# fritzsedlazeck/Sniffles

Measured on NVIDIA H100. Metric: aligned long-read Gbp/s through lead->cluster->consensus, higher is better.
Workload: dtype int32

## Files before the change

sniffles_b200/csrc/api.cu:

```cuda
#include <algorithm>
#include <climits>
#include <cstdio>
#include <cstdlib>
#include <cstring>
#include <string>
#include <vector>
#include <dlfcn.h>
#include <omp.h>

#include "common.cuh"
#include "prims.cuh"
#include "extract.cuh"
#include "cluster.cuh"
#include "consensus.cuh"
#include "poa.cuh"
#include "combine.cuh"
#include "population.cuh"
#include "ingest.cuh"
#include "bgzf_write.cuh"
#include "genotype.cuh"
#include "rnames.cuh"
#include "reference.cuh"

template <bool Pinned> struct Buf {
// ... 53 lines not shown

struct Caps { unsigned long long lead = 0, cand = 0, cand_lead = 0, rn = 0, alt = 0, scr16 = 0, item = 0, tile = 0, req = 0, req16 = 0; };

struct snfb_ctx {
    int device = 0; cudaStream_t st = nullptr, st_copy = nullptr, st_side = nullptr; cudaEvent_t ev_b = nullptr, ev_mid = nullptr, ev_fork = nullptr, ev_join = nullptr; std::string err;
    cudaEvent_t ev_aligned[consensus::MAX_SLICES] = {}, ev_slice[consensus::MAX_SLICES] = {}; int n_slices = consensus::DEFAULT_SLICES;
    snfb_config cfg{}; bool have_cfg = false;
    bool loaded = false, on_device = false, seq_on_demand = false; const uint8_t* h_seq = nullptr; uint32_t evt_min = 0;
    uint64_t n_rec = 0, n_cigar = 0, n_var = 0, n_seq = 0; uint32_t n_task = 0, n_contig = 0, n_tr = 0, n_mask = 0;
    const snfb_rec* d_rec = nullptr; const uint16_t* d_cigar = nullptr; const uint8_t* d_var = nullptr; const uint8_t* d_seq = nullptr;
    DevBuf b_rec, b_cigar, b_var, b_seq, b_task, b_contig, b_tr, b_trp, b_mask, b_mask_off, b_mask_task;
    HostBuf h_c16, h_rec16;
    DevBuf b_comp, b_raw, b_ing, b_ing_work; HostBuf h_ing; uint64_t ing_sizes[8] = {0, 0, 0, 0, 0, 0, 0, 0}; bool from_bam = false;
    DevBuf b_zin, b_zslot, b_zout, b_zwork;
    DevBuf b_gt;
    DevBuf b_rn, b_rn_text; HostBuf h_rn_meta, h_rn_text;
    DevBuf b_pop, b_popq; population::P pop{}; bool have_pop = false;
    DevBuf b_ref, b_ref_work; std::vector<refseq::Contig> ref_ctg; bool have_ref = false;
    HostBuf h_ref_runs, h_ref_coff, h_ref_out; uint64_t ref_n_runs = 0;
    std::vector<snfb_task> tasks;
    std::vector<snfb_region> regions, next_regions; DevBuf b_region; uint32_t n_region = 0; bool cov_view = false;
    Caps cap; bool force_no_cuts = false;
    DevBuf b_ctr, arena_r, arena_l, arena_c;
    int32_t* rec_pos; int32_t* rec_end; uint8_t* rec_flags; double* rec_nm; uint32_t* rec_nlead; uint32_t* rec_lead_off; uint32_t* sa_list; extract::RecScan* scanrec; extract::RecClip* clip; int32_t* rec_big;
    uint32_t* task_first; uint32_t* task_last; uint32_t* task_reads; unsigned long long* task_cov; int32_t* task_span; double* task_nm; double* nm_part; unsigned* nm_cnt; extract::Seg* sa_seg; uint32_t* scan_tmp_r;
    int32_t* v_pos; int32_t* v_end; uint8_t* v_flags; uint64_t* v_k0; uint64_t* v_k1; uint32_t* v_v0; uint32_t* v_v1; uint32_t* v_hist; uint32_t* v_scan; unsigned long long* v_n;
    snfb_lead* leads; extract::Event* ev_buf; snfb_lead* sorted_leads; uint32_t* radix_hist;
    cluster::B B{};
    consensus::C Cc{}; consensus::SeqReq* seq_req; uint32_t* arena_off; uint8_t* seq_arena; uint32_t* q_scan_tmp;
    HostBuf h_seq_req, h_seq_arena; uint64_t seq_h2d_bytes = 0;
    bool stage_a_done = false, stage_b_done = false, stage_c_done = false;
    HostBuf h_ctr_buf; DevCounters* h_mid = nullptr; DevCounters* h_fin = nullptr; consensus::Work* h_work = nullptr;
    HostBuf h_leads, h_task_reads, h_task_nm, h_rec_nm, h_cand, h_cand_leads, h_rnames, h_rn_off, h_task_cov, h_task_cov_raw, h_alt, h_cov_bins;
    void* comm = nullptr; int rank = 0, nranks = 1; DevBuf b_gsend, b_grecv; HostBuf h_gather, h_gather_out; unsigned long long gather_cap = 0;
    cudaEvent_t ev[MAX_TIMINGS + 1]; const char* ev_name[MAX_TIMINGS + 1]; uint64_t ev_bytes[MAX_TIMINGS + 1]; int n_ev = 0; int n_ev_load = 0; uint64_t launches = 0; uint64_t reruns = 0;
};

static uint32_t evt_need(const snfb_ctx* ctx) {
    if (!ctx->have_cfg) return SNFB_CIGAR16_EVT_MIN;
    int t = ctx->cfg.minsvlen_screen < 1 ? 1 : ctx->cfg.minsvlen_screen;
    if ((ctx->cfg.qc_nm_measure || ctx->cfg.phase) && t > 11) t = 11;
    return (uint32_t)(t < (int)SNFB_CIGAR16_EVT_MIN ? t : (int)SNFB_CIGAR16_EVT_MIN);
}
static void ctx_fail(snfb_ctx* ctx, const char* what, const char* msg) { ctx->err = std::string(what) + ": " + msg; }
static int fail(snfb_ctx* ctx, const std::string& m) { ctx->err = m; return 1; }

static void mark(snfb_ctx* ctx, const char* name, uint64_t bytes = 0) {
    if (ctx->n_ev >= MAX_TIMINGS) return;
    cudaEventRecord(ctx->ev[ctx->n_ev], ctx->st);
    ctx->ev_name[ctx->n_ev] = name; ctx->ev_bytes[ctx->n_ev] = bytes; ++ctx->n_ev;
}
static int grid_for(unsigned long long n, int threads) { unsigned long long g = (n + threads - 1) / threads; if (g < 1) g = 1; if (g > (uint64_t)NUM_SMS * 32) g = (uint64_t)NUM_SMS * 32; return (int)g; }
static int bits_for(uint32_t n) { int b = 0; while ((1ull << b) < n) ++b; return b; }

__global__ void k_gather_leads(const snfb_lead* __restrict__ leads, const uint32_t* __restrict__ sval, snfb_lead* __restrict__ out, const unsigned long long* n_ptr, unsigned long long cap) {
    const unsigned long long n = *n_ptr < cap ? *n_ptr : cap;
    for (unsigned long long i = blockIdx.x * (unsigned long long)blockDim.x + threadIdx.x; i < n; i += (unsigned long long)gridDim.x * blockDim.x) out[i] = leads[sval[i]];
}
__global__ void k_view_keys(const snfb_rec* __restrict__ rec, const int32_t* __restrict__ rec_pos, unsigned long long n, uint64_t* __restrict__ key, uint32_t* __restrict__ val, unsigned long long* n_out) {
    for (unsigned long long i = blockIdx.x * (unsigned long long)blockDim.x + threadIdx.x; i < n; i += (unsigned long long)gridDim.x * blockDim.x) {
        key[i] = ((uint64_t)(uint32_t)__ldg(&rec[i].task) << 32) | (uint64_t)((uint32_t)rec_pos[i] ^ 0x80000000u); val[i] = (uint32_t)i;
    }
    if (blockIdx.x == 0 && threadIdx.x == 0) *n_out = n;
}
__global__ void k_view_gather(const uint32_t* __restrict__ ord, unsigned long long n, const int32_t* __restrict__ pos, const int32_t* __restrict__ end, const uint8_t* __restrict__ flags,
                              int32_t* __restrict__ v_pos, int32_t* __restrict__ v_end, uint8_t* __restrict__ v_flags) {
    for (unsigned long long i = blockIdx.x * (unsigned long long)blockDim.x + threadIdx.x; i < n; i += (unsigned long long)gridDim.x * blockDim.x) {
        const uint32_t j = ord[i]; v_pos[i] = pos[j]; v_end[i] = end[j]; v_flags[i] = flags[j];
    }
}
__global__ void k_cov_bins(const int32_t* __restrict__ rec_pos, const int32_t* __restrict__ rec_end, const uint8_t* __restrict__ rec_flags, uint32_t lo, uint32_t hi,
                           int binsize, long long contig_len, long long nbins, unsigned long long* __restrict__ acc) {
    for (unsigned long long i = lo + blockIdx.x * (unsigned long long)blockDim.x + threadIdx.x; i < hi; i += (unsigned long long)gridDim.x * blockDim.x) {
        if (!(rec_flags[i] & extract::RF_PASS)) continue;
        long long a = rec_pos[i], e = rec_end[i]; if (a < 0) a = 0; if (e > contig_len) e = contig_len;
        if (e <= a) continue;
        for (long long bb = a / binsize; bb <= (e - 1) / binsize && bb < nbins; ++bb) {
            const long long s0 = bb * binsize, s1 = s0 + binsize;
            const long long o0 = a > s0 ? a : s0, o1 = e < s1 ? e : s1;
            if (o1 > o0) atomicAdd(&acc[bb], (unsigned long long)(o1 - o0));
        }
    }
}


struct GatherHdr { unsigned long long n_cand, n_alt, n_rn, n_leads, need_bytes, overflow, pad0, pad1; };
__host__ __device__ inline void gather_offsets(const GatherHdr& h, unsigned long long off[6]) {
    auto al = [](unsigned long long x) { return (x + 15ull) & ~15ull; };
    off[0] = sizeof(GatherHdr); off[1] = al(off[0] + h.n_cand * sizeof(snfb_cand)); off[2] = al(off[1] + h.n_alt); off[3] = al(off[2] + 8 * h.n_rn);
    off[4] = al(off[3] + 4 * h.n_cand); off[5] = al(off[4] + h.n_leads * sizeof(snfb_lead));
}
// ... 479 lines not shown
    CUDA_TRY(cudaStreamSynchronize(st));
    ctx->loaded = true; ctx->from_bam = true; return 0;
}

int snfb_ingest_sizes(snfb_ctx* ctx, uint64_t out[8]) {
    if (!ctx || !out || !ctx->from_bam) return 1;
    for (int i = 0; i < 8; ++i) out[i] = ctx->ing_sizes[i];
    return 0;
}
int snfb_ingest_fetch(snfb_ctx* ctx, snfb_rec* rec, uint16_t* cigar16, uint8_t* var, uint8_t* seq) {
    if (!ctx || !ctx->from_bam || !ctx->loaded) return ctx ? fail(ctx, "snfb_ingest_fetch: no block built by snfb_load_bam") : 1;
    cudaSetDevice(ctx->device);
    if (rec && ctx->n_rec) CUDA_TRY(cudaMemcpy(rec, ctx->d_rec, sizeof(snfb_rec) * ctx->n_rec, cudaMemcpyDeviceToHost));
    if (cigar16 && ctx->n_cigar) CUDA_TRY(cudaMemcpy(cigar16, ctx->d_cigar, 2 * ctx->n_cigar, cudaMemcpyDeviceToHost));
    if (var && ctx->n_var) CUDA_TRY(cudaMemcpy(var, ctx->d_var, ctx->n_var, cudaMemcpyDeviceToHost));
    if (seq && ctx->n_seq) CUDA_TRY(cudaMemcpy(seq, ctx->d_seq, ctx->n_seq, cudaMemcpyDeviceToHost));
    return 0;
}

}

static void carve_r(snfb_ctx* ctx, Carver& c) {
    const size_t n = ctx->n_rec + 1, nt = ctx->n_task;
    ctx->rec_pos = c.take<int32_t>(n); ctx->rec_end = c.take<int32_t>(n); ctx->rec_flags = c.take<uint8_t>(n); ctx->rec_nm = c.take<double>(n); ctx->rec_nlead = c.take<uint32_t>(n); ctx->rec_lead_off = c.take<uint32_t>(n);
    ctx->sa_list = c.take<uint32_t>(n); ctx->scanrec = c.take<extract::RecScan>(n); ctx->clip = c.take<extract::RecClip>(n); ctx->rec_big = c.take<int32_t>(n);
    ctx->task_first = c.take<uint32_t>(nt); ctx->task_last = c.take<uint32_t>(nt); ctx->task_reads = c.take<uint32_t>(nt); ctx->task_cov = c.take<unsigned long long>(nt); ctx->task_span = c.take<int32_t>(nt); ctx->task_nm = c.take<double>(nt);
    const size_t cpt = (ctx->n_rec + extract::NM_CHUNK - 1) / extract::NM_CHUNK + 1;
    ctx->nm_part = c.take<double>(cpt * nt + 1); ctx->nm_cnt = c.take<unsigned>(cpt * nt + 1);
    ctx->sa_seg = c.take<extract::Seg>((size_t)extract::MAXSEG * extract::SA_THREADS * extract::SA_BLOCKS);
    ctx->scan_tmp_r = c.take<uint32_t>(prims::scan_tmp_elems(n) + 16);
    const size_t nv = ctx->cov_view ? n : 1;
    ctx->v_pos = c.take<int32_t>(nv); ctx->v_end = c.take<int32_t>(nv); ctx->v_flags = c.take<uint8_t>(nv);
    ctx->v_k0 = c.take<uint64_t>(nv); ctx->v_k1 = c.take<uint64_t>(nv); ctx->v_v0 = c.take<uint32_t>(nv); ctx->v_v1 = c.take<uint32_t>(nv);
    ctx->v_hist = c.take<uint32_t>(prims::radix_hist_elems(nv) + 16); ctx->v_scan = c.take<uint32_t>(prims::scan_tmp_elems(std::max<size_t>(nv, prims::radix_hist_elems(nv))) + 16);
    ctx->v_n = c.take<unsigned long long>(1);
}
static void carve_l(snfb_ctx* ctx, Carver& c) {
    const size_t n = (size_t)ctx->cap.lead + 8; cluster::B& b = ctx->B;
    ctx->leads = c.take<snfb_lead>(n); ctx->ev_buf = c.take<extract::Event>(n); ctx->sorted_leads = c.take<snfb_lead>(n);
    b.key0 = c.take<uint64_t>(n); b.val0 = c.take<uint32_t>(n); b.key1 = c.take<uint64_t>(n); b.val1 = c.take<uint32_t>(n); b.flag = c.take<uint32_t>(n); b.scan = c.take<uint32_t>(n);
    b.scan_tmp = c.take<uint32_t>(prims::scan_tmp_elems(std::max<unsigned long long>(n, prims::radix_hist_elems(n))) + 16);
    ctx->radix_hist = c.take<uint32_t>(prims::radix_hist_elems(n) + 16);
    b.bin_start = c.take<uint32_t>(n); b.bin_nl = c.take<uint32_t>(n); b.bin_nlong = c.take<uint32_t>(n); b.bin_kept = c.take<uint32_t>(n); b.bin_hap = c.take<uint32_t>(3 * n);
    b.kl_off = c.take<uint32_t>(n); b.kll_off = c.take<uint32_t>(n); b.kb_idx = c.take<uint32_t>(n); b.kl = c.take<uint32_t>(n); b.kll = c.take<uint32_t>(n); b.kleads = c.take<snfb_lead>(n); b.klleads = c.take<snfb_lead>(n);
    b.kb_bin = c.take<uint32_t>(n); b.kb_lead_off = c.take<uint32_t>(n); b.kb_lead_n = c.take<uint32_t>(n); b.kb_long_off = c.take<uint32_t>(n); b.kb_long_n = c.take<uint32_t>(n); b.kb_seed = c.take<int32_t>(n); b.kb_chain = c.take<uint32_t>(n); b.kb_repeat = c.take<uint8_t>(n);
    b.seg_start = c.take<uint32_t>(n); b.c_next = c.take<uint32_t>(n); b.c_last = c.take<uint32_t>(n); b.c_sd = c.take<double>(n); b.c_mean = c.take<double>(n); b.c_rep = c.take<uint8_t>(n);
    b.seg_sd_last = c.take<double>(n); b.seg_maxsd_first = c.take<double>(n); b.cl_first = c.take<uint32_t>(n); b.cl_last = c.take<uint32_t>(n); b.cl_rep = c.take<uint8_t>(n); b.big_list = c.take<uint32_t>(n); b.mid_list = c.take<uint32_t>(n);
// ... 5 lines not shown
static void carve_c(snfb_ctx* ctx, Carver& c) {
    const Caps& k = ctx->cap; cluster::B& b = ctx->B; consensus::C& cc = ctx->Cc;
    b.cand = c.take<snfb_cand>(k.cand + 1); b.cand_leads = c.take<snfb_lead>(k.cand_lead + 1); b.out_plo = c.take<uint32_t>(k.cand_lead + 1); b.out_pn = c.take<uint32_t>(k.cand_lead + 1);
    b.rnames = c.take<uint64_t>(k.rn + 1); b.rn_off_out = c.take<uint32_t>(k.cand + 2);
    cc.plan_best = c.take<uint32_t>(k.cand + 1); cc.plan_nother = c.take<uint32_t>(k.cand + 1); cc.plan_otot = c.take<uint32_t>(k.cand + 1); cc.alt_len = c.take<uint32_t>(k.cand + 1); cc.scr_len = c.take<uint32_t>(k.cand + 1);
    cc.alt_off = c.take<uint32_t>(k.cand + 1); cc.scr_off = c.take<uint32_t>(k.cand + 1); cc.work_big = c.take<uint32_t>(k.cand + 1); cc.work_small = c.take<uint32_t>(k.cand + 1); cc.work = c.take<consensus::Work>(1);
    cc.q_cnt = c.take<uint32_t>(consensus::NQ * (k.cand + 1)); cc.q_off = c.take<uint32_t>(consensus::NQ * (k.cand + 1)); ctx->q_scan_tmp = c.take<uint32_t>(consensus::NQ * prims::scan_tmp_elems(k.cand));
    cc.items_big = c.take<consensus::C::Item>(k.item + 1); cc.items_small = c.take<consensus::C::Item>(k.item + 1); cc.tiles = c.take<uint2>(k.tile + 1);
    cc.alt = c.take<uint8_t>(k.alt + 64); cc.scr = c.take<uint8_t>(k.scr16 * 16 + 64);
    ctx->seq_req = c.take<consensus::SeqReq>(k.req + 1); ctx->seq_arena = c.take<uint8_t>(k.req16 * 16 + 64);
}
static int ensure_arenas(snfb_ctx* ctx) {
    if (carve(ctx->arena_r, [&](Carver& c) { carve_r(ctx, c); })) return fail(ctx, "out of device memory (per-record arrays)");
    if (carve(ctx->arena_l, [&](Carver& c) { carve_l(ctx, c); })) return fail(ctx, "out of device memory (per-lead arrays)");
    if (carve(ctx->arena_c, [&](Carver& c) { carve_c(ctx, c); })) return fail(ctx, "out of device memory (candidate / consensus arrays)");
    return 0;
}

static void bind_inputs(snfb_ctx* ctx) {
    cluster::B& b = ctx->B;
    b.leads = ctx->leads; b.rec = ctx->d_rec; b.task = ctx->b_task.as<snfb_task>(); b.contig = ctx->b_contig.as<snfb_contig>();
    b.tr = ctx->n_tr ? ctx->b_tr.as<int32_t>() : nullptr; b.tr_pmax = ctx->b_trp.as<int32_t>();
    b.rec_pos = ctx->cov_view ? ctx->v_pos : ctx->rec_pos; b.rec_end = ctx->cov_view ? ctx->v_end : ctx->rec_end; b.rec_flags = ctx->cov_view ? ctx->v_flags : ctx->rec_flags; b.rec_nm = ctx->rec_nm; b.rec_nlead = ctx->rec_nlead; b.rec_lead_off = ctx->rec_lead_off;
    b.task_first = ctx->task_first; b.task_last = ctx->task_last; b.task_maxspan = ctx->task_span;
    b.mask = ctx->n_mask ? ctx->b_mask.as<int32_t>() : nullptr; b.mask_task_off = ctx->n_mask ? ctx->b_mask_off.as<uint32_t>() : nullptr;
    b.n_task = ctx->n_task; b.n_bound = ctx->cap.lead; b.ctr = ctx->b_ctr.as<DevCounters>(); b.cfg = ctx->cfg;
    b.cut_gap = ctx->force_no_cuts ? INT_MAX : cluster::break_gap(ctx->cfg);
    b.cand_cap = ctx->cap.cand; b.cand_lead_cap = ctx->cap.cand_lead; b.rn_cap = ctx->cap.rn;
    consensus::C& c = ctx->Cc;
    c.cand = b.cand; c.cand_rw = b.cand; c.cand_leads = b.cand_leads; c.out_plo = b.out_plo; c.out_pn = b.out_pn; c.ord = b.ord; c.kleads = b.kleads; c.rec = ctx->d_rec; c.seq = ctx->d_seq; c.arena_off = nullptr;
    c.cand_cap = ctx->cap.cand; c.ctr = b.ctr; c.cfg = ctx->cfg; c.item_cap = ctx->cap.item; c.tile_cap = ctx->cap.tile; c.alt_cap = ctx->cap.alt; c.scr_cap16 = ctx->cap.scr16;
}

static int enqueue_stage_a(snfb_ctx* ctx) {
    const uint64_t nrec = ctx->n_rec; const uint32_t nt = ctx->n_task; const snfb_config& cf = ctx->cfg; cluster::B& b = ctx->B;
    DevCounters* ctr = b.ctr; cudaStream_t st = ctx->st;
    CUDA_TRY(cudaMemsetAsync(ctr, 0, sizeof(DevCounters), st));
    CUDA_TRY(cudaMemsetAsync(ctx->task_first, 0, 4 * nt, st)); CUDA_TRY(cudaMemsetAsync(ctx->task_last, 0, 4 * nt, st));
    CUDA_TRY(cudaMemsetAsync(ctx->task_reads, 0, 4 * nt, st)); CUDA_TRY(cudaMemsetAsync(ctx->task_cov, 0, 8 * nt, st)); CUDA_TRY(cudaMemsetAsync(ctx->task_span, 0, 4 * nt, st));
    CUDA_TRY(cudaMemsetAsync(ctx->task_nm, 0, 8 * nt, st));
    extract::WalkParams S{};
    S.scan = ctx->scanrec; S.n_rec = (uint32_t)nrec; S.cigar = ctx->d_cigar; S.task = b.task;
    S.rec_end = ctx->rec_end; S.rec_nlead = ctx->rec_nlead; S.rec_big = ctx->rec_big; S.rec = ctx->d_rec; S.region = dev_regions(ctx);
    S.ev = ctx->ev_buf; S.ev_cap = ctx->cap.lead; S.n_ev = &ctr->n_ev; S.ctr = ctr; S.minsv = cf.minsvlen_screen;
    if (evt_need(ctx) < ctx->evt_min) {
        if (ctx->on_device) return fail(ctx, "the device-resident CIGAR16 arena was packed with a larger event length than the configuration needs: repack with snfb_pack_cigar16(evt_min)");
        launch(ctx->launches, extract::k_reflag, NUM_SMS * 8, 256, 0, st, const_cast<uint16_t*>(ctx->d_cigar), ctx->n_cigar, evt_need(ctx));
// ... 18 lines not shown
        launch(ctx->launches, extract::k_rec_post, (unsigned)((nrec + 255) / 256), 256, 0, st, Q);
        mark(ctx, "k_emit");
        extract::EmitParams E{};
        E.rec = ctx->d_rec; E.clip = ctx->clip; E.var = ctx->d_var; E.ev = S.ev; E.n_ev = S.n_ev; E.ev_cap = ctx->cap.lead;
        E.leads = ctx->leads; E.ctr = ctr; E.maxlen = cf.dev_seq_cache_maxlen; E.detect_large_ins = cf.detect_large_ins; E.longinslen = (double)cf.long_ins_length / 2.0;
        launch(ctx->launches, extract::k_emit, NUM_SMS * 16, 128, 0, st, E);
        mark(ctx, "k_sa");
        extract::SaParams A{};
        A.rec = ctx->d_rec; A.clip = ctx->clip; A.var = ctx->d_var; A.task = b.task; A.contig = b.contig; A.n_contig = ctx->n_contig;
        A.sa_list = ctx->sa_list; A.n_sa = &ctr->n_sa; A.rec_end = ctx->rec_end; A.rec_nlead = ctx->rec_nlead; A.leads = E.leads; A.lead_cap = ctx->cap.lead; A.ctr = ctr; A.cfg = cf; A.seg_scratch = ctx->sa_seg; A.region = dev_regions(ctx);
        launch(ctx->launches, extract::k_sa, extract::SA_BLOCKS, extract::SA_THREADS, 0, st, A);
        mark(ctx, "k_task_nm");
        const int cpt = (int)((nrec + extract::NM_CHUNK - 1) / extract::NM_CHUNK);
        launch(ctx->launches, extract::k_nm_partial, dim3(cpt, nt), 256, 0, st, ctx->rec_flags, ctx->rec_nm, ctx->task_first, ctx->task_last, ctx->nm_part, ctx->nm_cnt);
        launch(ctx->launches, extract::k_task_nm, nt, 256, 0, st, ctx->task_first, ctx->task_last, ctx->nm_part, ctx->nm_cnt, cpt, ctx->task_nm);
        if (ctx->cov_view) {
            mark(ctx, "cov_order");
            launch(ctx->launches, k_view_keys, grid_for(nrec, 256), 256, 0, st, ctx->d_rec, ctx->rec_pos, (unsigned long long)nrec, ctx->v_k0, ctx->v_v0, ctx->v_n);
            prims::RadixTemp vt{ ctx->v_hist, ctx->v_scan };
            bool vfirst = true;
            prims::radix_sort(ctx->launches, ctx->v_k0, ctx->v_v0, ctx->v_k1, ctx->v_v1, vt, ctx->v_n, nrec, 32 + bits_for(nt), &vfirst, st);
            launch(ctx->launches, k_view_gather, grid_for(nrec, 256), 256, 0, st, vfirst ? ctx->v_v0 : ctx->v_v1, (unsigned long long)nrec, ctx->rec_pos, ctx->rec_end, ctx->rec_flags, ctx->v_pos, ctx->v_end, ctx->v_flags);
        }
    }
    mark(ctx, "scan_rec_leads");
    prims::exclusive_scan(ctx->launches, ctx->rec_nlead, ctx->rec_lead_off, ctx->scan_tmp_r, nullptr, nrec, &ctr->n_leads, st);
    const unsigned long long nb = b.n_bound; const int g = grid_for(nb, 256);
    mark(ctx, "sort_leads");
    launch(ctx->launches, cluster::k_scatter_keys, g, 256, 0, st, b);
    prims::RadixTemp rt{ ctx->radix_hist, b.scan_tmp };
    bool first = true;
    prims::radix_sort(ctx->launches, b.key0, b.val0, b.key1, b.val1, rt, &ctr->n_leads, nb, cluster::TASK_SHIFT + bits_for(ctx->n_task), &first, st);
    b.skey = first ? b.key0 : b.key1; b.sval = first ? b.val0 : b.val1;
    mark(ctx, "bins");
    launch(ctx->launches, cluster::k_bin_heads, g, 256, 0, st, b);
    prims::exclusive_scan(ctx->launches, b.flag, b.scan, b.scan_tmp, &ctr->n_leads, nb, &ctr->n_bins, st);
    launch(ctx->launches, cluster::k_bin_build, g, 256, 0, st, b);
    launch(ctx->launches, cluster::k_bin_stats, g, 256, 0, st, b);
    mark(ctx, nullptr);
    CUDA_TRY(cudaGetLastError());
    return 0;
}

static int enqueue_stage_b(snfb_ctx* ctx) {
    cluster::B& b = ctx->B; DevCounters* ctr = b.ctr; cudaStream_t st = ctx->st;
    const unsigned long long nb = b.n_bound; const int g = grid_for(nb, 128);
// ... 928 lines not shown
```

sniffles_b200/csrc/cluster.cuh:

```cuda
#pragma once
#include "common.cuh"
#include "extract.cuh"

namespace cluster {

constexpr int TYPE_SHIFT = 26;
constexpr int TASK_SHIFT = 29;
constexpr uint32_t NONE = 0xffffffffu;
constexpr int SMALL_CAP = 48;
constexpr int WARP_CAP = 128;
constexpr int BLOCK_CAP = 1024;

struct B {
    snfb_lead* leads; const snfb_rec* rec; const snfb_task* task; const snfb_contig* contig; const int32_t* tr; const int32_t* tr_pmax;
    const int32_t* rec_pos; const int32_t* rec_end; const uint8_t* rec_flags; const double* rec_nm; const uint32_t* rec_nlead; const uint32_t* rec_lead_off;
    const uint32_t* task_first; const uint32_t* task_last; const int32_t* task_maxspan;
    const int32_t* mask; const uint32_t* mask_task_off;
    uint32_t n_task; unsigned long long n_bound;
    DevCounters* ctr;
    snfb_config cfg;
    int cut_gap;
    uint64_t* key0; uint32_t* val0; uint64_t* key1; uint32_t* val1;
    const uint64_t* skey; const uint32_t* sval;
    uint32_t* flag; uint32_t* scan;
    uint32_t* bin_start; uint32_t* bin_nl; uint32_t* bin_nlong; uint32_t* bin_kept; uint32_t* bin_hap;
    uint32_t* kl_off; uint32_t* kll_off; uint32_t* kb_idx;
    uint32_t* kl; uint32_t* kll; snfb_lead* kleads; snfb_lead* klleads;
    uint32_t* kb_bin; uint32_t* kb_lead_off; uint32_t* kb_lead_n; uint32_t* kb_long_off; uint32_t* kb_long_n; int32_t* kb_seed; uint32_t* kb_chain; uint8_t* kb_repeat;
    uint32_t* seg_start;
    uint32_t* c_next; uint32_t* c_last; double* c_sd; double* c_mean; uint8_t* c_rep;
    double* seg_sd_last; double* seg_maxsd_first;
    uint32_t* cl_first; uint32_t* cl_last; uint8_t* cl_rep;
    uint32_t* big_list; uint32_t* mid_list;
    uint64_t* g_khi; uint64_t* g_klo; uint32_t* g_u32;
    uint32_t* ord;
    snfb_lead* st_leads; uint32_t* st_plo; uint32_t* st_pn; uint64_t* st_rn; snfb_cand* cand_tmp; uint8_t* sub_valid;
    uint32_t* cl_nsub; uint32_t* cl_nvalid; uint32_t* cl_nlead; uint32_t* cl_nrn; uint32_t* cl_cand_base; uint32_t* cl_lead_base; uint32_t* cl_rn_base;
    snfb_cand* cand; snfb_lead* cand_leads; uint32_t* out_plo; uint32_t* out_pn; uint64_t* rnames; uint32_t* rn_off_out;
    unsigned long long cand_cap, cand_lead_cap, rn_cap;
// ... 723 lines not shown
            if (id >= b.cand_cap || (unsigned long long)lout + n + nl > b.cand_lead_cap || (unsigned long long)rout + cd.support > b.rn_cap) { if (lane == 0) atomicAdd(&b.ctr->scratch_overflow, 1ULL); ++id; lout += n + nl; rout += cd.support; continue; }
            { const uint4* s = reinterpret_cast<const uint4*>(b.st_leads + st0); uint4* d = reinterpret_cast<uint4*>(b.cand_leads + lout);
              for (int i = lane; i < n * 4; i += 32) d[i] = s[i]; }
            { const uint4* s = reinterpret_cast<const uint4*>(b.klleads + llo); uint4* d = reinterpret_cast<uint4*>(b.cand_leads + lout + n);
              for (int i = lane; i < nl * 4; i += 32) d[i] = s[i]; }
            for (int i = lane; i < n; i += 32) { b.out_plo[lout + i] = b.st_plo[st0 + i]; b.out_pn[lout + i] = b.st_pn[st0 + i]; }
            for (int i = lane; i < nl; i += 32) { b.out_plo[lout + n + i] = NONE; b.out_pn[lout + n + i] = 0; }
            for (int i = lane; i < nq && i < cd.support; i += 32) b.rnames[rout + i] = b.st_rn[st0 + i];
            __syncwarp();
            if (lane == 0) {
                if (cd.svtype == SNFB_INS && cd.svlen >= b.cfg.long_ins_length && cd.support > nq) {
                    int o = nq < cd.support ? nq : cd.support;
                    for (int i = 0; i < nl && o < cd.support; ++i) { const uint64_t h = b.klleads[llo + i].qname_hash; bool dup = false; for (int q = 0; q < o; ++q) if (b.rnames[rout + q] == h) { dup = true; break; } if (!dup) b.rnames[rout + o++] = h; }
                    hsort1(b.rnames + rout, o);
                }
                cd.lead_off = (int)lout; cd.long_off = (int)(lout + n);
                b.cand[id] = cd; b.rn_off_out[id] = rout;
            }
            ++id; lout += n + nl; rout += cd.support;
        }
    }
}

__device__ inline void cover_count_warp(const B& b, int t, long long p, uint32_t out[3]) {
    out[0] = out[1] = out[2] = 0;
    const uint32_t lo = b.task_first[t], hi = b.task_last[t];
    if (lo >= hi) return;
    uint32_t a = lo, z = hi;
    while (a < z) { uint32_t mid = a + ((z - a) >> 1); if ((long long)b.rec_pos[mid] <= p) a = mid + 1; else z = mid; }
    const long long span = b.task_maxspan[t];
    uint32_t c0 = 0, c1 = 0, c2 = 0;
    for (long long i = (long long)a - 1 - lane_id(); i >= (long long)lo; i -= 32) {
        const long long ps = b.rec_pos[i]; if (ps + span <= p) break;
        const uint8_t f = b.rec_flags[i];
        if ((f & extract::RF_PASS) && (long long)b.rec_end[i] > p) { const int h = (f >> 2) & 3; c0 += h == 0; c1 += h == 1; c2 += h == 2; }
    }
    out[0] = __reduce_add_sync(FULL, c0); out[1] = __reduce_add_sync(FULL, c1); out[2] = __reduce_add_sync(FULL, c2);
}
__device__ inline void cov_at_warp(const B& b, int t, long long idx, int* out) {
    const long long L = b.task[t].contig_len;
    if (idx < 0) idx += L;
    if (idx < 0 || idx >= L) return;
    if (b.mask) {
        uint32_t lo = b.mask_task_off[t], hi = b.mask_task_off[t + 1];
        while (lo < hi) { const uint32_t mid = lo + ((hi - lo) >> 1); if ((long long)b.mask[2 * mid + 1] <= idx) lo = mid + 1; else hi = mid; }
        if (lo < b.mask_task_off[t + 1] && (long long)b.mask[2 * lo] <= idx && idx >= b.task[t].start && idx < b.task[t].end) { *out = 0; return; }
    }
    uint32_t c[3]; cover_count_warp(b, t, idx, c); *out = (int)((c[0] + c[1] + c[2]) & 0xffffu);
}

struct CovSv { int task, svtype; long long pos, svlen; int bnd_is_first; };
template <class At, class Prev> __device__ inline bool cov_probes(long long i, At at, Prev prev, long long bs, long long ud, long long p[5]) {
    const CovSv c = at(i); long long start = c.pos, end; bool ok = true;
    if (c.svtype == SNFB_INS) end = start + 1;
    else if (c.svtype == SNFB_BND) {
        if (c.bnd_is_first) start -= 1;
        const long long j = prev(i);
        if (j >= 0) { const CovSv q = at(j); end = q.svtype == SNFB_INS ? q.pos + 1 : q.pos + (q.svlen < 0 ? -q.svlen : q.svlen); }
        else { end = start; ok = false; }
    } else end = c.pos + (c.svlen < 0 ? -c.svlen : c.svlen);
    if (c.svtype == SNFB_INS || c.svtype == SNFB_BND) { p[1] = start - bs; p[2] = start; p[3] = end + bs; }
    else { p[1] = start; p[2] = (long long)__ddiv_rn((double)(start + end), 2.0); p[3] = end - bs; }
    p[0] = start - ud; p[4] = end + ud;
    return ok;
}

__global__ void k_coverage(B b) {
    const unsigned long long nc = b.ctr->n_cand < b.cand_cap ? b.ctr->n_cand : b.cand_cap;
    const long long bs = b.cfg.coverage_binsize, ud = (long long)b.cfg.coverage_binsize * b.cfg.coverage_updown_bins;
    const unsigned long long nw = ((unsigned long long)gridDim.x * blockDim.x) >> 5;
    const auto at = [&](long long j) { const snfb_cand& q = b.cand[j]; return CovSv{ q.task, q.svtype, q.pos, q.svlen, q.bnd_is_first }; };
    const auto prev = [&](long long i) {
        const int t = b.cand[i].task; long long j = i - 1; while (j >= 0 && b.cand[j].task == t && b.cand[j].svtype == SNFB_BND) --j;
        return j >= 0 && b.cand[j].task == t ? j : -1ll; };
    for (unsigned long long i = ((unsigned long long)blockIdx.x * blockDim.x + threadIdx.x) >> 5; i < nc; i += nw) {
        snfb_cand* c = &b.cand[i]; const int t = c->task;
        long long p[5];
        if (!cov_probes((long long)i, at, prev, bs, ud, p) && lane_id() == 0) atomicAdd(&b.ctr->soft_errors, 1ULL);
        int v[5] = { 0, 0, 0, 0, 0 };
        for (int k = 0; k < 5; ++k) cov_at_warp(b, t, p[k], &v[k]);
        uint32_t hr[3]; const int cb = b.cfg.cluster_binsize; cover_count_warp(b, t, (long long)(c->cluster_seed / cb) * cb + cb - 1, hr);
        if (lane_id() == 0) {
            c->cov_upstream = v[0]; c->cov_start = v[1]; c->cov_center = v[2]; c->cov_end = v[3]; c->cov_downstream = v[4];
            for (int h = 0; h < 3; ++h) c->hap_counts[3 + h] = (int)(hr[h] > 65535u ? 65535u : hr[h]);
        }
    }
}

__device__ inline void mask_run(const B& b, int t, unsigned long long m, long long* a, long long* e) {
    const long long L = b.task[t].contig_len;
    *a = b.mask[2 * m]; *e = b.mask[2 * m + 1];
    if (*a < b.task[t].start) *a = b.task[t].start; if (*e > b.task[t].end) *e = b.task[t].end; if (*a < 0) *a = 0; if (*e > L) *e = L;
}
template <class F> __device__ inline void pass_overlaps_warp(const B& b, int t, long long a, long long e, F f) {
    const uint32_t lo = b.task_first[t], hi = b.task_last[t];
    if (a >= e || lo >= hi) return;
    const long long L = b.task[t].contig_len;
    uint32_t x = lo, z = hi;
    while (x < z) { const uint32_t mid = x + ((z - x) >> 1); if ((long long)b.rec_pos[mid] < e) x = mid + 1; else z = mid; }
    const long long span = b.task_maxspan[t];
    for (long long i = (long long)x - 1 - lane_id(); i >= (long long)lo; i -= 32) {
        const long long ps = b.rec_pos[i]; if (ps + span <= a) break;
        if (!(b.rec_flags[i] & extract::RF_PASS)) continue;
        long long re = b.rec_end[i]; if (re > L) re = L;
        const long long o0 = ps > a ? ps : a, o1 = re < e ? re : e;
        if (o1 > o0) f(o0, o1);
    }
}

__global__ void k_mask_bp(B b, const uint32_t* __restrict__ mask_task, uint32_t n_mask, unsigned long long* task_cov_bp) {
    const unsigned long long nw = ((unsigned long long)gridDim.x * blockDim.x) >> 5;
    for (unsigned long long m = ((unsigned long long)blockIdx.x * blockDim.x + threadIdx.x) >> 5; m < n_mask; m += nw) {
        const int t = (int)mask_task[m]; long long a, e; mask_run(b, t, m, &a, &e);
        unsigned long long sum = 0;
        pass_overlaps_warp(b, t, a, e, [&](long long o0, long long o1) { sum += (unsigned long long)(o1 - o0); });
        #pragma unroll
        for (int o = 16; o; o >>= 1) sum += __shfl_xor_sync(FULL, sum, o);
        if (lane_id() == 0 && sum) atomicAdd(&task_cov_bp[t], 0ull - sum);
    }
}

__global__ void k_mask_bins(B b, int t, int binsize, unsigned long long* acc) {
    const unsigned long long nw = ((unsigned long long)gridDim.x * blockDim.x) >> 5;
    const uint32_t m0 = b.mask_task_off[t], m1 = b.mask_task_off[t + 1];
    for (unsigned long long m = m0 + (((unsigned long long)blockIdx.x * blockDim.x + threadIdx.x) >> 5); m < m1; m += nw) {
        long long a, e; mask_run(b, t, m, &a, &e);
// ... 12 lines not shown
```

sniffles_b200/csrc/prims.cuh:

```cuda
#pragma once
#include "common.cuh"

namespace prims {

constexpr int SCAN_THREADS = 256;
constexpr int SCAN_ITEMS = 16;
constexpr int SCAN_TILE = SCAN_THREADS * SCAN_ITEMS;

__device__ __forceinline__ uint32_t warp_incl_scan(uint32_t v) {
    #pragma unroll
    for (int o = 1; o < 32; o <<= 1) { uint32_t t = __shfl_up_sync(FULL, v, o); if (lane_id() >= o) v += t; }
    return v;
}

__device__ inline uint32_t block_excl_scan(uint32_t v, uint32_t* total) {
    __shared__ uint32_t wsum[8];
    __shared__ uint32_t tot;
    uint32_t inc = warp_incl_scan(v);
    int w = threadIdx.x >> 5;
    if (lane_id() == 31) wsum[w] = inc;
    __syncthreads();
    if (threadIdx.x < 32) {
        uint32_t x = threadIdx.x < 8 ? wsum[threadIdx.x] : 0;
        uint32_t xi = warp_incl_scan(x);
// ... 34 lines not shown
    in += blockIdx.y * stride; out += blockIdx.y * stride; tile_sum += (size_t)blockIdx.y * gridDim.x;
    unsigned long long base = (unsigned long long)blockIdx.x * SCAN_TILE + (unsigned long long)threadIdx.x * SCAN_ITEMS;
    uint32_t v[SCAN_ITEMS]; uint32_t s = 0;
    #pragma unroll
    for (int i = 0; i < SCAN_ITEMS; ++i) { v[i] = base + i < n ? in[base + i] : 0; s += v[i]; }
    uint32_t tot; uint32_t e = block_excl_scan(s, &tot) + tile_sum[blockIdx.x];
    #pragma unroll
    for (int i = 0; i < SCAN_ITEMS; ++i) { if (base + i < n) out[base + i] = e; e += v[i]; }
}

inline void exclusive_scan_cols(uint64_t& launches, const uint32_t* in, uint32_t* out, size_t stride, int cols, uint32_t* tmp, const unsigned long long* n_ptr,
                                unsigned long long n_bound, unsigned long long* total_out, cudaStream_t st) {
    if (n_bound == 0) { if (total_out) cudaMemsetAsync(total_out, 0, 8 * cols, st); return; }
    int ntiles = (int)((n_bound + SCAN_TILE - 1) / SCAN_TILE);
    launch(launches, k_scan_reduce, dim3(ntiles, cols), SCAN_THREADS, 0, st, in, tmp, n_ptr, n_bound, stride);
    launch(launches, k_scan_tiles, cols, SCAN_THREADS, 0, st, tmp, ntiles, total_out);
    launch(launches, k_scan_down, dim3(ntiles, cols), SCAN_THREADS, 0, st, in, out, tmp, n_ptr, n_bound, stride);
}
inline void exclusive_scan(uint64_t& launches, const uint32_t* in, uint32_t* out, uint32_t* tmp, const unsigned long long* n_ptr, unsigned long long n_bound,
                           unsigned long long* total_out, cudaStream_t st) {
    exclusive_scan_cols(launches, in, out, 0, 1, tmp, n_ptr, n_bound, total_out, st);
}
inline size_t scan_tmp_elems(unsigned long long n_bound) { return (size_t)((n_bound + SCAN_TILE - 1) / SCAN_TILE) + 1; }

constexpr int RS_THREADS = 256;
constexpr int RS_ITEMS = 8;
constexpr int RS_TILE = RS_THREADS * RS_ITEMS;

__global__ void __launch_bounds__(RS_THREADS) k_radix_hist(const uint64_t* __restrict__ keys, uint32_t* __restrict__ hist, const unsigned long long* __restrict__ n_ptr,
                                                           unsigned long long n_bound, int shift, int nblk) {
    __shared__ uint32_t h[256];
    unsigned long long n = *n_ptr; if (n > n_bound) n = n_bound;
    unsigned long long base = (unsigned long long)blockIdx.x * RS_TILE;
    h[threadIdx.x] = 0;
    __syncthreads();
    if (base < n) {
        #pragma unroll
        for (int i = 0; i < RS_ITEMS; ++i) { unsigned long long j = base + (unsigned long long)i * RS_THREADS + threadIdx.x; if (j < n) atomicAdd(&h[(keys[j] >> shift) & 255], 1u); }
    }
    __syncthreads();
    hist[(size_t)threadIdx.x * nblk + blockIdx.x] = h[threadIdx.x];
}

__global__ void __launch_bounds__(RS_THREADS) k_radix_scatter(const uint64_t* __restrict__ kin, const uint32_t* __restrict__ vin, uint64_t* __restrict__ kout, uint32_t* __restrict__ vout,
                                                              const uint32_t* __restrict__ offs, const unsigned long long* __restrict__ n_ptr, unsigned long long n_bound, int shift, int nblk) {
    __shared__ uint32_t cnt[8][256];
// ... 56 lines not shown
```

Baseline: 10260.

## Bound coverage windows with per-task segmented prefix max of read ends

Adds a segmented max-scan over read end positions, segmented by task, so each record carries the running maximum end within its task. Coverage queries now binary-search both the start bound (first record whose running end exceeds the probe) and the end bound (first record starting after the probe), replacing the backward walk bounded by the task's max span. The per-candidate coverage kernel also batches its six probes into one warp: lanes compute the six windows in parallel and the warp sweeps their union once. This costs three extra scan kernels plus a head-bitmap pass and extra memory, and aims to cut scanned records when long reads inflate the max span.

```diff
diff --git a/sniffles_b200/csrc/api.cu b/sniffles_b200/csrc/api.cu
--- a/sniffles_b200/csrc/api.cu
+++ b/sniffles_b200/csrc/api.cu
@@ -99,7 +99,7 @@
     std::vector<snfb_region> regions, next_regions; DevBuf b_region; uint32_t n_region = 0; bool cov_view = false;
     Caps cap; bool force_no_cuts = false;
     DevBuf b_ctr, arena_r, arena_l, arena_c;
-    int32_t* rec_pos; int32_t* rec_end; uint8_t* rec_flags; double* rec_nm; uint32_t* rec_nlead; uint32_t* rec_lead_off; uint32_t* sa_list; extract::RecScan* scanrec; extract::RecClip* clip; int32_t* rec_big;
+    int32_t* rec_pos; int32_t* rec_end; int32_t* rec_endmax; uint32_t* rec_heads; prims::SegMax* endmax_tmp; uint8_t* rec_flags; double* rec_nm; uint32_t* rec_nlead; uint32_t* rec_lead_off; uint32_t* sa_list; extract::RecScan* scanrec; extract::RecClip* clip; int32_t* rec_big;
     uint32_t* task_first; uint32_t* task_last; uint32_t* task_reads; unsigned long long* task_cov; int32_t* task_span; double* task_nm; double* nm_part; unsigned* nm_cnt; extract::Seg* sa_seg; uint32_t* scan_tmp_r;
     int32_t* v_pos; int32_t* v_end; uint8_t* v_flags; uint64_t* v_k0; uint64_t* v_k1; uint32_t* v_v0; uint32_t* v_v1; uint32_t* v_hist; uint32_t* v_scan; unsigned long long* v_n;
     snfb_lead* leads; extract::Event* ev_buf; snfb_lead* sorted_leads; uint32_t* radix_hist;
@@ -144,6 +144,12 @@
                               int32_t* __restrict__ v_pos, int32_t* __restrict__ v_end, uint8_t* __restrict__ v_flags) {
     for (unsigned long long i = blockIdx.x * (unsigned long long)blockDim.x + threadIdx.x; i < n; i += (unsigned long long)gridDim.x * blockDim.x) {
         const uint32_t j = ord[i]; v_pos[i] = pos[j]; v_end[i] = end[j]; v_flags[i] = flags[j];
+    }
+}
+__global__ void k_task_heads(const uint32_t* __restrict__ first, const uint32_t* __restrict__ last, uint32_t nt, uint32_t* __restrict__ heads) {
+    for (uint32_t t = blockIdx.x * blockDim.x + threadIdx.x; t < nt; t += gridDim.x * blockDim.x) {
+        const uint32_t lo = first[t];
+        if (lo < last[t]) atomicOr(&heads[lo >> 5], 1u << (lo & 31));
     }
 }
 __global__ void k_cov_bins(const int32_t* __restrict__ rec_pos, const int32_t* __restrict__ rec_end, const uint8_t* __restrict__ rec_flags, uint32_t lo, uint32_t hi,
@@ -669,7 +675,9 @@
 
 static void carve_r(snfb_ctx* ctx, Carver& c) {
     const size_t n = ctx->n_rec + 1, nt = ctx->n_task;
-    ctx->rec_pos = c.take<int32_t>(n); ctx->rec_end = c.take<int32_t>(n); ctx->rec_flags = c.take<uint8_t>(n); ctx->rec_nm = c.take<double>(n); ctx->rec_nlead = c.take<uint32_t>(n); ctx->rec_lead_off = c.take<uint32_t>(n);
+    ctx->rec_pos = c.take<int32_t>(n); ctx->rec_end = c.take<int32_t>(n); ctx->rec_endmax = c.take<int32_t>(n);
+    ctx->rec_heads = c.take<uint32_t>(prims::segmax_head_words(n)); ctx->endmax_tmp = c.take<prims::SegMax>(prims::segmax_tmp_elems(n));
+    ctx->rec_flags = c.take<uint8_t>(n); ctx->rec_nm = c.take<double>(n); ctx->rec_nlead = c.take<uint32_t>(n); ctx->rec_lead_off = c.take<uint32_t>(n);
     ctx->sa_list = c.take<uint32_t>(n); ctx->scanrec = c.take<extract::RecScan>(n); ctx->clip = c.take<extract::RecClip>(n); ctx->rec_big = c.take<int32_t>(n);
     ctx->task_first = c.take<uint32_t>(nt); ctx->task_last = c.take<uint32_t>(nt); ctx->task_reads = c.take<uint32_t>(nt); ctx->task_cov = c.take<unsigned long long>(nt); ctx->task_span = c.take<int32_t>(nt); ctx->task_nm = c.take<double>(nt);
     const size_t cpt = (ctx->n_rec + extract::NM_CHUNK - 1) / extract::NM_CHUNK + 1;
@@ -721,7 +729,7 @@
     b.leads = ctx->leads; b.rec = ctx->d_rec; b.task = ctx->b_task.as<snfb_task>(); b.contig = ctx->b_contig.as<snfb_contig>();
     b.tr = ctx->n_tr ? ctx->b_tr.as<int32_t>() : nullptr; b.tr_pmax = ctx->b_trp.as<int32_t>();
     b.rec_pos = ctx->cov_view ? ctx->v_pos : ctx->rec_pos; b.rec_end = ctx->cov_view ? ctx->v_end : ctx->rec_end; b.rec_flags = ctx->cov_view ? ctx->v_flags : ctx->rec_flags; b.rec_nm = ctx->rec_nm; b.rec_nlead = ctx->rec_nlead; b.rec_lead_off = ctx->rec_lead_off;
-    b.task_first = ctx->task_first; b.task_last = ctx->task_last; b.task_maxspan = ctx->task_span;
+    b.task_first = ctx->task_first; b.task_last = ctx->task_last; b.task_maxspan = ctx->task_span; b.rec_endmax = ctx->rec_endmax;
     b.mask = ctx->n_mask ? ctx->b_mask.as<int32_t>() : nullptr; b.mask_task_off = ctx->n_mask ? ctx->b_mask_off.as<uint32_t>() : nullptr;
     b.n_task = ctx->n_task; b.n_bound = ctx->cap.lead; b.ctr = ctx->b_ctr.as<DevCounters>(); b.cfg = ctx->cfg;
     b.cut_gap = ctx->force_no_cuts ? INT_MAX : cluster::break_gap(ctx->cfg);
@@ -786,6 +794,10 @@
             prims::radix_sort(ctx->launches, ctx->v_k0, ctx->v_v0, ctx->v_k1, ctx->v_v1, vt, ctx->v_n, nrec, 32 + bits_for(nt), &vfirst, st);
             launch(ctx->launches, k_view_gather, grid_for(nrec, 256), 256, 0, st, vfirst ? ctx->v_v0 : ctx->v_v1, (unsigned long long)nrec, ctx->rec_pos, ctx->rec_end, ctx->rec_flags, ctx->v_pos, ctx->v_end, ctx->v_flags);
         }
+        mark(ctx, "cov_endmax", 12 * nrec);
+        CUDA_TRY(cudaMemsetAsync(ctx->rec_heads, 0, 4 * prims::segmax_head_words(nrec + 1), st));
+        launch(ctx->launches, k_task_heads, grid_for(nt, 256), 256, 0, st, ctx->task_first, ctx->task_last, nt, ctx->rec_heads);
+        prims::segmented_max_scan(ctx->launches, b.rec_end, ctx->rec_heads, ctx->rec_endmax, ctx->endmax_tmp, nrec, st);
     }
     mark(ctx, "scan_rec_leads");
     prims::exclusive_scan(ctx->launches, ctx->rec_nlead, ctx->rec_lead_off, ctx->scan_tmp_r, nullptr, nrec, &ctr->n_leads, st);
diff --git a/sniffles_b200/csrc/cluster.cuh b/sniffles_b200/csrc/cluster.cuh
--- a/sniffles_b200/csrc/cluster.cuh
+++ b/sniffles_b200/csrc/cluster.cuh
@@ -15,6 +15,7 @@
     snfb_lead* leads; const snfb_rec* rec; const snfb_task* task; const snfb_contig* contig; const int32_t* tr; const int32_t* tr_pmax;
     const int32_t* rec_pos; const int32_t* rec_end; const uint8_t* rec_flags; const double* rec_nm; const uint32_t* rec_nlead; const uint32_t* rec_lead_off;
     const uint32_t* task_first; const uint32_t* task_last; const int32_t* task_maxspan;
+    const int32_t* rec_endmax;
     const int32_t* mask; const uint32_t* mask_task_off;
     uint32_t n_task; unsigned long long n_bound;
     DevCounters* ctr;
@@ -784,30 +785,44 @@
     }
 }
 
+__device__ __forceinline__ uint32_t first_above(const int32_t* a, uint32_t lo, uint32_t hi, long long p) {
+    while (lo < hi) { const uint32_t mid = lo + ((hi - lo) >> 1); if ((long long)a[mid] <= p) lo = mid + 1; else hi = mid; }
+    return lo;
+}
+__device__ __forceinline__ uint32_t window_bound(const B& b, int lane, uint32_t lo, uint32_t hi, long long p) {
+    return first_above(lane & 1 ? b.rec_pos : b.rec_endmax, lo, hi, p);
+}
+__device__ __forceinline__ void cover_window_warp(const B& b, uint32_t lo, uint32_t hi, long long p, uint32_t* s, uint32_t* z) {
+    const uint32_t x = window_bound(b, lane_id(), lo, hi, p);
+    *s = __shfl_sync(FULL, x, 0); *z = __shfl_sync(FULL, x, 1);
+}
+
 __device__ inline void cover_count_warp(const B& b, int t, long long p, uint32_t out[3]) {
     out[0] = out[1] = out[2] = 0;
     const uint32_t lo = b.task_first[t], hi = b.task_last[t];
     if (lo >= hi) return;
-    uint32_t a = lo, z = hi;
-    while (a < z) { uint32_t mid = a + ((z - a) >> 1); if ((long long)b.rec_pos[mid] <= p) a = mid + 1; else z = mid; }
-    const long long span = b.task_maxspan[t];
+    uint32_t s, z; cover_window_warp(b, lo, hi, p, &s, &z);
     uint32_t c0 = 0, c1 = 0, c2 = 0;
-    for (long long i = (long long)a - 1 - lane_id(); i >= (long long)lo; i -= 32) {
-        const long long ps = b.rec_pos[i]; if (ps + span <= p) break;
-        const uint8_t f = b.rec_flags[i];
-        if ((f & extract::RF_PASS) && (long long)b.rec_end[i] > p) { const int h = (f >> 2) & 3; c0 += h == 0; c1 += h == 1; c2 += h == 2; }
+    for (uint32_t i = s + lane_id(); i < z; i += 32) {
+        const uint8_t f = b.rec_flags[i]; const long long pe = b.rec_end[i];
+        if ((f & extract::RF_PASS) && pe > p) { const int h = (f >> 2) & 3; c0 += h == 0; c1 += h == 1; c2 += h == 2; }
     }
     out[0] = __reduce_add_sync(FULL, c0); out[1] = __reduce_add_sync(FULL, c1); out[2] = __reduce_add_sync(FULL, c2);
 }
-__device__ inline void cov_at_warp(const B& b, int t, long long idx, int* out) {
+__device__ inline long long cov_index(const B& b, int t, long long idx) {
     const long long L = b.task[t].contig_len;
     if (idx < 0) idx += L;
-    if (idx < 0 || idx >= L) return;
+    if (idx < 0 || idx >= L) return -1;
     if (b.mask) {
         uint32_t lo = b.mask_task_off[t], hi = b.mask_task_off[t + 1];
         while (lo < hi) { const uint32_t mid = lo + ((hi - lo) >> 1); if ((long long)b.mask[2 * mid + 1] <= idx) lo = mid + 1; else hi = mid; }
-        if (lo < b.mask_task_off[t + 1] && (long long)b.mask[2 * lo] <= idx && idx >= b.task[t].start && idx < b.task[t].end) { *out = 0; return; }
-    }
+        if (lo < b.mask_task_off[t + 1] && (long long)b.mask[2 * lo] <= idx && idx >= b.task[t].start && idx < b.task[t].end) return -1;
+    }
+    return idx;
+}
+__device__ inline void cov_at_warp(const B& b, int t, long long idx, int* out) {
+    idx = cov_index(b, t, idx);
+    if (idx < 0) { *out = 0; return; }
     uint32_t c[3]; cover_count_warp(b, t, idx, c); *out = (int)((c[0] + c[1] + c[2]) & 0xffffu);
 }
 
@@ -835,14 +850,52 @@
     const auto prev = [&](long long i) {
         const int t = b.cand[i].task; long long j = i - 1; while (j >= 0 && b.cand[j].task == t && b.cand[j].svtype == SNFB_BND) --j;
         return j >= 0 && b.cand[j].task == t ? j : -1ll; };
+    const int lane = lane_id(), k = lane >> 1;
     for (unsigned long long i = ((unsigned long long)blockIdx.x * blockDim.x + threadIdx.x) >> 5; i < nc; i += nw) {
         snfb_cand* c = &b.cand[i]; const int t = c->task;
-        long long p[5];
-        if (!cov_probes((long long)i, at, prev, bs, ud, p) && lane_id() == 0) atomicAdd(&b.ctr->soft_errors, 1ULL);
-        int v[5] = { 0, 0, 0, 0, 0 };
-        for (int k = 0; k < 5; ++k) cov_at_warp(b, t, p[k], &v[k]);
-        uint32_t hr[3]; const int cb = b.cfg.cluster_binsize; cover_count_warp(b, t, (long long)(c->cluster_seed / cb) * cb + cb - 1, hr);
-        if (lane_id() == 0) {
+        long long p[6];
+        if (!cov_probes((long long)i, at, prev, bs, ud, p) && lane == 0) atomicAdd(&b.ctr->soft_errors, 1ULL);
+        const int cb = b.cfg.cluster_binsize; p[5] = (long long)(c->cluster_seed / cb) * cb + cb - 1;
+        const uint32_t lo = b.task_first[t], hi = b.task_last[t];
+        long long q = p[0];
+        #pragma unroll
+        for (int j = 1; j < 6; ++j) q = j == k ? p[j] : q;
+        if (k < 5) q = cov_index(b, t, q);
+        const bool on = k == 5 || (k < 5 && q >= 0);
+        uint32_t x = hi;
+        if (on && lo < hi) x = window_bound(b, lane, lo, hi, q);
+        uint32_t s = __shfl_sync(FULL, x, (2 * lane) & 31), z = __shfl_sync(FULL, x, (2 * lane + 1) & 31);
+        if (lane >= 6 || z < s) z = s;
+        long long pk[6]; unsigned act = __ballot_sync(FULL, on && (lane & 1) == 0);
+        #pragma unroll
+        for (int j = 0; j < 6; ++j) pk[j] = __shfl_sync(FULL, q, 2 * j);
+        act = ((act & 0x1u) | ((act >> 1) & 0x2u) | ((act >> 2) & 0x4u) | ((act >> 3) & 0x8u) | ((act >> 4) & 0x10u) | ((act >> 5) & 0x20u));
+        uint32_t n5[5] = { 0, 0, 0, 0, 0 }, h3[3] = { 0, 0, 0 };
+        uint32_t done = 0;
+        for (;;) {
+            const bool live = z > (s > done ? s : done);
+            const uint32_t gs = __reduce_min_sync(FULL, live ? (s > done ? s : done) : 0xffffffffu);
+            if (gs == 0xffffffffu) break;
+            uint32_t gz = gs;
+            for (;;) { const uint32_t nz = __reduce_max_sync(FULL, live && s <= gz ? z : 0u); if (nz <= gz) break; gz = nz; }
+            #pragma unroll 2
+            for (uint32_t r = gs + lane; r < gz; r += 32) {
+                const uint8_t f = b.rec_flags[r]; const long long ps = b.rec_pos[r], pe = b.rec_end[r];
+                if (!(f & extract::RF_PASS)) continue;
+                const int h = (f >> 2) & 3;
+                #pragma unroll
+                for (int j = 0; j < 5; ++j) n5[j] += ((act >> j) & 1u) && ps <= pk[j] && pe > pk[j] && h < 3;
+                if ((act >> 5) & 1u && ps <= pk[5] && pe > pk[5]) { h3[0] += h == 0; h3[1] += h == 1; h3[2] += h == 2; }
+            }
+            done = gz;
+        }
+        int v[5];
+        #pragma unroll
+        for (int j = 0; j < 5; ++j) v[j] = (int)(__reduce_add_sync(FULL, n5[j]) & 0xffffu);
+        uint32_t hr[3];
+        #pragma unroll
+        for (int h = 0; h < 3; ++h) hr[h] = __reduce_add_sync(FULL, h3[h]);
+        if (lane == 0) {
             c->cov_upstream = v[0]; c->cov_start = v[1]; c->cov_center = v[2]; c->cov_end = v[3]; c->cov_downstream = v[4];
             for (int h = 0; h < 3; ++h) c->hap_counts[3 + h] = (int)(hr[h] > 65535u ? 65535u : hr[h]);
         }
@@ -858,12 +911,11 @@
     const uint32_t lo = b.task_first[t], hi = b.task_last[t];
     if (a >= e || lo >= hi) return;
     const long long L = b.task[t].contig_len;
-    uint32_t x = lo, z = hi;
-    while (x < z) { const uint32_t mid = x + ((z - x) >> 1); if ((long long)b.rec_pos[mid] < e) x = mid + 1; else z = mid; }
-    const long long span = b.task_maxspan[t];
-    for (long long i = (long long)x - 1 - lane_id(); i >= (long long)lo; i -= 32) {
-        const long long ps = b.rec_pos[i]; if (ps + span <= a) break;
+    const uint32_t x = window_bound(b, lane_id(), lo, hi, lane_id() & 1 ? e - 1 : a);
+    const uint32_t s = __shfl_sync(FULL, x, 0), z = __shfl_sync(FULL, x, 1);
+    for (uint32_t i = s + lane_id(); i < z; i += 32) {
         if (!(b.rec_flags[i] & extract::RF_PASS)) continue;
+        const long long ps = b.rec_pos[i];
         long long re = b.rec_end[i]; if (re > L) re = L;
         const long long o0 = ps > a ? ps : a, o1 = re < e ? re : e;
         if (o1 > o0) f(o0, o1);
diff --git a/sniffles_b200/csrc/prims.cuh b/sniffles_b200/csrc/prims.cuh
--- a/sniffles_b200/csrc/prims.cuh
+++ b/sniffles_b200/csrc/prims.cuh
@@ -80,6 +80,101 @@
     exclusive_scan_cols(launches, in, out, 0, 1, tmp, n_ptr, n_bound, total_out, st);
 }
 inline size_t scan_tmp_elems(unsigned long long n_bound) { return (size_t)((n_bound + SCAN_TILE - 1) / SCAN_TILE) + 1; }
+
+struct SegMax { uint32_t f; int32_t v; };
+__device__ __forceinline__ SegMax segmax_op(SegMax a, SegMax b) { return { a.f | b.f, b.f ? b.v : (a.v > b.v ? a.v : b.v) }; }
+__device__ inline SegMax block_segmax_excl(SegMax x, SegMax* total) {
+    __shared__ SegMax wt[8];
+    __shared__ SegMax tot;
+    const SegMax id{ 0u, -1 };
+    SegMax inc = x;
+    #pragma unroll
+    for (int o = 1; o < 32; o <<= 1) {
+        const SegMax p{ __shfl_up_sync(FULL, inc.f, o), __shfl_up_sync(FULL, inc.v, o) };
+        if (lane_id() >= o) inc = segmax_op(p, inc);
+    }
+    const int w = threadIdx.x >> 5;
+    if (lane_id() == 31) wt[w] = inc;
+    __syncthreads();
+    if (threadIdx.x < 32) {
+        SegMax y = threadIdx.x < 8 ? wt[threadIdx.x] : id;
+        #pragma unroll
+        for (int o = 1; o < 8; o <<= 1) {
+            const SegMax p{ __shfl_up_sync(FULL, y.f, o), __shfl_up_sync(FULL, y.v, o) };
+            if (lane_id() >= o) y = segmax_op(p, y);
+        }
+        const SegMax e{ __shfl_up_sync(FULL, y.f, 1), __shfl_up_sync(FULL, y.v, 1) };
+        if (threadIdx.x < 8) wt[threadIdx.x] = threadIdx.x ? e : id;
+        if (threadIdx.x == 7) tot = y;
+    }
+    __syncthreads();
+    SegMax ex{ __shfl_up_sync(FULL, inc.f, 1), __shfl_up_sync(FULL, inc.v, 1) };
+    if (lane_id() == 0) ex = id;
+    const SegMax r = segmax_op(wt[w], ex);
+    *total = tot;
+    __syncthreads();
+    return r;
+}
+__device__ __forceinline__ uint32_t segmax_load(const int32_t* __restrict__ in, const uint32_t* __restrict__ heads, unsigned long long base,
+                                                unsigned long long n, int32_t v[SCAN_ITEMS]) {
+    static_assert(SCAN_ITEMS == 16, "one 16-bit slice of a head word, four 16-byte loads");
+    #pragma unroll
+    for (int i = 0; i < SCAN_ITEMS; ++i) v[i] = -1;
+    if (base >= n) return 0u;
+    #pragma unroll
+    for (int q = 0; q < SCAN_ITEMS / 4; ++q) {
+        const int4 x = __ldg(reinterpret_cast<const int4*>(in + base) + q);
+        v[4 * q] = x.x; v[4 * q + 1] = x.y; v[4 * q + 2] = x.z; v[4 * q + 3] = x.w;
+    }
+    #pragma unroll
+    for (int i = 0; i < SCAN_ITEMS; ++i) if (base + i >= n) v[i] = -1;
+    return (heads[base >> 5] >> (base & 31)) & ((1u << SCAN_ITEMS) - 1u);
+}
+__device__ __forceinline__ SegMax segmax_fold(const int32_t v[SCAN_ITEMS], uint32_t h) {
+    SegMax a{ h, -1 };
+    #pragma unroll
+    for (int i = 0; i < SCAN_ITEMS; ++i) a.v = ((h >> i) & 1u) ? v[i] : (a.v > v[i] ? a.v : v[i]);
+    return a;
+}
+__global__ void __launch_bounds__(SCAN_THREADS) k_segmax_reduce(const int32_t* __restrict__ in, const uint32_t* __restrict__ heads, SegMax* __restrict__ tile, unsigned long long n) {
+    const unsigned long long base = (unsigned long long)blockIdx.x * SCAN_TILE + (unsigned long long)threadIdx.x * SCAN_ITEMS;
+    int32_t v[SCAN_ITEMS]; const uint32_t h = segmax_load(in, heads, base, n, v);
+    SegMax tot; block_segmax_excl(segmax_fold(v, h), &tot);
+    if (threadIdx.x == 0) tile[blockIdx.x] = tot;
+}
+__global__ void __launch_bounds__(SCAN_THREADS) k_segmax_tiles(SegMax* __restrict__ tile, int ntiles) {
+    SegMax carry{ 0u, -1 };
+    for (int b = 0; b < ntiles; b += SCAN_THREADS) {
+        const int j = b + threadIdx.x; SegMax tot;
+        const SegMax e = block_segmax_excl(j < ntiles ? tile[j] : SegMax{ 0u, -1 }, &tot);
+        if (j < ntiles) tile[j] = segmax_op(carry, e);
+        carry = segmax_op(carry, tot);
+    }
+}
+__global__ void __launch_bounds__(SCAN_THREADS) k_segmax_down(const int32_t* __restrict__ in, const uint32_t* __restrict__ heads, const SegMax* __restrict__ tile,
+                                                              int32_t* __restrict__ out, unsigned long long n) {
+    const unsigned long long base = (unsigned long long)blockIdx.x * SCAN_TILE + (unsigned long long)threadIdx.x * SCAN_ITEMS;
+    int32_t v[SCAN_ITEMS]; const uint32_t h = segmax_load(in, heads, base, n, v);
+    SegMax tot; int32_t run = segmax_op(tile[blockIdx.x], block_segmax_excl(segmax_fold(v, h), &tot)).v;
+    #pragma unroll
+    for (int i = 0; i < SCAN_ITEMS; ++i) { run = ((h >> i) & 1u) ? v[i] : (run > v[i] ? run : v[i]); v[i] = run; }
+    if (base + SCAN_ITEMS <= n) {
+        #pragma unroll
+        for (int q = 0; q < SCAN_ITEMS / 4; ++q) reinterpret_cast<int4*>(out + base)[q] = make_int4(v[4 * q], v[4 * q + 1], v[4 * q + 2], v[4 * q + 3]);
+    } else {
+        #pragma unroll
+        for (int i = 0; i < SCAN_ITEMS; ++i) if (base + i < n) out[base + i] = v[i];
+    }
+}
+inline void segmented_max_scan(uint64_t& launches, const int32_t* in, const uint32_t* heads, int32_t* out, SegMax* tmp, unsigned long long n, cudaStream_t st) {
+    if (n == 0) return;
+    const int ntiles = (int)((n + SCAN_TILE - 1) / SCAN_TILE);
+    launch(launches, k_segmax_reduce, ntiles, SCAN_THREADS, 0, st, in, heads, tmp, n);
+    launch(launches, k_segmax_tiles, 1, SCAN_THREADS, 0, st, tmp, ntiles);
+    launch(launches, k_segmax_down, ntiles, SCAN_THREADS, 0, st, in, heads, tmp, out, n);
+}
+inline size_t segmax_tmp_elems(unsigned long long n) { return (size_t)((n + SCAN_TILE - 1) / SCAN_TILE) + 1; }
+inline size_t segmax_head_words(unsigned long long n) { return segmax_tmp_elems(n) * (SCAN_TILE / 32); }
 
 constexpr int RS_THREADS = 256;
 constexpr int RS_ITEMS = 8;
```

New measurement: 10430 (median of 6 runs). 1.02x the previous value.
